# pingcap/tidb

Measured on NVIDIA H100. Metric: hash-join probe rows/sec, higher is better.
Workload: dtype int64

## Files before the change

### tidb_b200/csrc/join.cu

```cuda
#include <memory>
#include <deque>
#include <algorithm>
#include <cmath>
#include <condition_variable>
#include "join_kernels.cuh"
#include "partition_kernels.cuh"
#include "chunk_io.cuh"

namespace tg {

static const int64_t kGeneralBatchRows = 16ll << 20;
static const int64_t kDirectPushRows = 128ll << 10;
static const int64_t kNextWindowRows = 1ll << 20;

struct Side {
  int ncols = 0;
  std::vector<int> types;
  std::vector<uint32_t> flags;
  std::vector<int> elem;
  std::vector<int> kelem;
  bool has_cells = false;
  std::vector<char> needed;
  int key_col = -1;
  std::vector<int> key_cols;
  std::vector<int> key_reject;
  std::vector<int> used;
  DevFilter filter{};
};

struct ColStore {
  std::vector<std::unique_ptr<DevBuf>> data, nulls;
  std::vector<char> has_nulls;
  int64_t rows = 0, cap_rows = 0;
  void init(int ncols) {
    data.clear(); nulls.clear();
    for (int i = 0; i < ncols; i++) { data.emplace_back(new DevBuf()); nulls.emplace_back(new DevBuf()); }
    has_nulls.assign(ncols, 0);
    rows = cap_rows = 0;
  }
  DevCols view(const Side& s) const {
    DevCols v{};
    for (int c = 0; c < s.ncols && c < TG_MAX_COLS; c++) {
      v.data[c] = s.needed[c] ? data[c]->p : nullptr;
      v.nulls[c] = (s.needed[c] && has_nulls[c]) ? nulls[c]->as<uint8_t>() : nullptr;
      v.elem_len[c] = s.elem[c];
    }
    return v;
  }
};

struct ResultBatch {
  std::vector<std::unique_ptr<DevBuf>> cols, bitmaps;
  int64_t rows = 0;
  int64_t consumed = 0;
};

}

using namespace tg;

struct JoinImpl;

struct tg_join {
  std::mutex mu;
  std::mutex res_mu;
  std::condition_variable res_cv;
  std::atomic<bool> closed{false};
  JoinImpl* impl = nullptr;
};

struct JoinImpl : DeviceHandle {
  std::mutex& res_mu;
  std::condition_variable& res_cv;
  explicit JoinImpl(tg_join& shell) : res_mu(shell.res_mu), res_cv(shell.res_cv) {}
  cudaStream_t d2h_stream = nullptr;
  double load_factor = 0.5;
  bool default_load_factor = true;

  int join_type = 0;
  bool build_is_right = true;
  Side build, probe;
  int n_lused = 0, n_rused = 0;
  std::vector<int> lused, rused;
  int probe_kind = PK_INNER;
  bool need_scan = false;
  int scan_mode = 0;
  bool has_flag_col = false;
  int n_out = 0;
  std::vector<int> out_elem;
  std::vector<int> kout_elem;
  KeySpec build_key{}, probe_key{};
  bool multi_key = false;
  DevBuf bkey_syn, bkey_syn_nn, pkey_syn, pkey_syn_nn;
  std::vector<tg_other_item> other;
  std::vector<int> other_build_cols;
  DevOther dev_other{};

  HostStage bstage;
  ColStore bcols;
  bool built = false;
  DevBuf table, rows_store, row_slot, row_rank, slot_used, scalars;
  TableView tv{};
  RowSpec rowspec{};
  std::vector<int> build_word_of_col;
  int u1_payload_col = -1;

  HostStage pstage;
  ColStore pcols_dev;
  DevBuf tmp_cnt, tmp_slot, tmp_off, tmp_sums, out_cursor;
  DevBuf part_scratch;
  DevBuf tile_cnt;
  double seg_match = 1.0;
  int seg_parts = 0;
  int64_t seg_rows = 0, seg_fill_max = 0;
  std::unique_ptr<DevBuf> part_cols[1 + TG_FAST_MAX_PCOLS];
  std::vector<std::unique_ptr<DevBuf>> tmp_valid;
  std::deque<std::unique_ptr<ResultBatch>> results;
  std::vector<std::unique_ptr<ResultBatch>> free_batches;
  std::unique_ptr<ResultBatch> dev_result;
  DevBuf iota;
  int64_t iota_rows = 0;
  std::vector<std::unique_ptr<DevBuf>> out_ids;
  std::atomic<bool> probe_finished{false};
  std::atomic<int64_t> d2h_bytes{0};
  PinBuf win;
  int64_t win_lo = 0, win_hi = 0;
  ResultBatch* win_batch = nullptr;

  tg_join_stats stats{};
};

namespace tg {

static int fill_side(Side& s, int n, const int32_t* types, const uint32_t* flags) {
  if (n <= 0 || n > TG_MAX_COLS) return fail(TG_ERR_UNSUPPORTED, "child schema must have 1..16 columns");
  s.ncols = n;
  s.types.assign(types, types + n);
  s.flags.resize(n);
  for (int i = 0; i < n; i++) s.flags[i] = flags ? flags[i] : 0;
  s.elem.resize(n);
  for (int i = 0; i < n; i++) s.elem[i] = fixed_len(types[i]);
  s.kelem.resize(n);
  for (int i = 0; i < n; i++) s.kelem[i] = s.elem[i] == kCellBytes ? 8 : s.elem[i];
  s.needed.assign(n, 0);
  return TG_OK;
}

static int key_kind_of(int tp) {
  if (is_int_family(tp)) return KEY_I64;
  if (tp == TG_TYPE_DOUBLE) return KEY_F64;
  if (tp == TG_TYPE_FLOAT) return KEY_F32;
  if (tp == TG_TYPE_DATE || tp == TG_TYPE_DATETIME || tp == TG_TYPE_TIMESTAMP) return KEY_TIME;
  return -1;
}
static bool key_unsigned(int tp, uint32_t flag) {
  if (tp == TG_TYPE_YEAR) return true;
  if (tp == TG_TYPE_DURATION) return false;
  return (flag & TG_FLAG_UNSIGNED) != 0;
}

static int check_filter(const Side& s, const tg_filter_item* items, int n, DevFilter& out) {
  if (n < 0 || n > TG_MAX_FILTER) return fail(TG_ERR_UNSUPPORTED, "at most 8 CNF filter items are offloaded");
  out.n = n;
  if (n > 0 && !items) return fail(TG_ERR_INVALID, "filter items are NULL");
  for (int i = 0; i < n; i++) {
    const tg_filter_item& it = items[i];
    if (it.lhs_col < 0 || it.lhs_col >= s.ncols || it.rhs_col >= s.ncols) return fail(TG_ERR_INVALID, "filter column out of range");
    const bool lreal = s.types[it.lhs_col] == TG_TYPE_DOUBLE;
    if ((it.is_real != 0) != lreal || (it.rhs_col >= 0 && (s.types[it.rhs_col] == TG_TYPE_DOUBLE) != lreal))
      return fail(TG_ERR_UNSUPPORTED, "filter compares columns of different families (the planner casts before the filter)");
    if (s.elem[it.lhs_col] != 8 || (it.rhs_col >= 0 && s.elem[it.rhs_col] != 8))
      return fail(TG_ERR_UNSUPPORTED, "filters are offloaded on 8-byte columns only");
    if (it.op < TG_CMP_LT || it.op > TG_CMP_NE) return fail(TG_ERR_INVALID, "bad filter op");
    out.items[i] = it;
  }
  return TG_OK;
}

static int setup(JoinImpl* j, const tg_join_desc* d) {
  if (!d) return fail(TG_ERR_INVALID, "desc is NULL");
  j->join_type = d->join_type;
  j->build_is_right = d->build_is_right != 0;
  Side left, right;
  TG_TRY(fill_side(left, d->n_left_cols, d->left_types, d->left_flags));
  TG_TRY(fill_side(right, d->n_right_cols, d->right_types, d->right_flags));
// ... 152 lines not shown
      TG_TRY(cs.nulls[c]->ensure_preserve(j->device, need, cs.has_nulls[c] ? had : 0, j->stream));
      if (!cs.has_nulls[c]) { TG_CUDA(cudaMemsetAsync(cs.nulls[c]->p, 0xff, had, j->stream)); cs.has_nulls[c] = 1; }
      if (chk->cols[c].null_bitmap) TG_CUDA(cudaMemcpyAsync(cs.nulls[c]->as<uint8_t>() + had, chk->cols[c].null_bitmap, (size_t)((n + 7) / 8), cudaMemcpyDeviceToDevice, j->stream));
      else TG_CUDA(cudaMemsetAsync(cs.nulls[c]->as<uint8_t>() + had, 0xff, (size_t)((n + 7) / 8), j->stream));
    }
  }
  cs.rows += n;
  return TG_OK;
}

static int probe_view(JoinImpl* j, const tg_chunk* chk, DevCols& v) {
  const Side& s = j->probe;
  TG_TRY(device_view(chk, s.ncols, s.needed, s.elem, v));
  for (int c = 0; c < s.ncols; c++)
    if (s.needed[c] && s.elem[c] == kCellBytes && (reinterpret_cast<uintptr_t>(v.data[c]) & 7)) return fail(TG_ERR_INVALID, "DECIMAL device columns must be 8-byte aligned");
  return TG_OK;
}

static int composite_key(JoinImpl* j, const Side& s, const DevCols& v, int64_t n, DevBuf& key, DevBuf& not_null) {
  TG_TRY(key.ensure(j->device, (size_t)(n + 1) * 8 + 16));
  TG_TRY(not_null.ensure(j->device, (size_t)((n + 31) / 32) * 4 + 16));
  if (n <= 0) return TG_OK;
  MultiKeySrc src{};
  src.nk = (int)s.key_cols.size();
  for (int q = 0; q < src.nk; q++) {
    const int c = s.key_cols[q];
    src.data[q] = reinterpret_cast<const int64_t*>(v.data[c]);
    src.nulls[q] = v.nulls[c];
    src.reject[q] = s.key_reject[q];
    if (!src.data[q]) return fail(TG_ERR_INVALID, "key column data is NULL");
  }
  k_composite_key<<<grid_size(j->nsm, n, 256, 8), 256, 0, j->stream>>>(src, n, key.as<int64_t>(), not_null.as<uint32_t>());
  j->stats.kernel_launches++;
  return TG_OK;
}

static int ensure_iota(JoinImpl* j, int64_t rows) {
  if (rows <= j->iota_rows) return TG_OK;
  rows = std::max(rows, 2 * j->iota_rows);
  TG_TRY(j->iota.ensure(j->device, (size_t)rows * 8 + 16));
  k_iota<<<grid_size(j->nsm, rows, 256, 8), 256, 0, j->stream>>>(j->iota.as<int64_t>(), rows);
  j->stats.kernel_launches++;
  j->iota_rows = rows;
  return TG_OK;
}

static int kernel_view(JoinImpl* j, const Side& s, DevCols& v, int64_t rows) {
  if (!s.has_cells) return TG_OK;
  TG_TRY(ensure_iota(j, rows));
  for (int c = 0; c < s.ncols; c++)
    if (s.needed[c] && s.elem[c] == kCellBytes) { v.data[c] = j->iota.p; v.elem_len[c] = 8; }
  return TG_OK;
}

struct ProbeTuning { int ctas_per_sm; bool partition; int parts; int part_min_mb; int part_min_rows; int inplace; };
static ProbeTuning probe_tuning() {
  ProbeTuning t;
  t.ctas_per_sm = env_int("TG_PROBE_CTAS_PER_SM", 0);
  t.partition = env_int("TG_PROBE_PARTITION", 1) != 0;
  t.parts = env_int("TG_PROBE_PARTS", 0);
  t.part_min_mb = env_int("TG_PROBE_PART_MIN_MB", 64);
  t.part_min_rows = env_int("TG_PROBE_PART_MIN_ROWS", 1 << 22);
  t.inplace = env_int("TG_PROBE_INPLACE", -1);
  return t;
}

static size_t l2_slice_target(int device) {
  static size_t cache[64];
  if (device >= 0 && device < 64 && cache[device]) return cache[device];
  int l2 = 0;
  if (cudaDeviceGetAttribute(&l2, cudaDevAttrL2CacheSize, device) != cudaSuccess || l2 <= 0) { cudaGetLastError(); l2 = 50 << 20; }
  const size_t t = (size_t)l2 / 4;
  if (device >= 0 && device < 64) cache[device] = t;
  return t;
}
static int probe_slices(size_t table_bytes, int device, int parts_override) {
  if (parts_override > 0) return std::min(parts_override, TG_MAX_PARTS);
  const size_t target = l2_slice_target(device);
  return (int)std::min<size_t>((table_bytes + target - 1) / target, TG_MAX_PARTS);
}
static const double kMaxDenseLoad = 0.5;
static const double kInplaceMinMatch = 0.995;

static int64_t inplace_seg_cap(const JoinImpl* j, int P, int64_t n_main, int64_t C0) {
  if (j->seg_parts != P || j->seg_rows <= 0) return C0;
  const double f = (double)j->seg_fill_max * (double)n_main / (double)j->seg_rows;
  const int64_t C = ((int64_t)(f + 8.0 * std::sqrt(f)) + 4096 + 127) / 128 * 128;
  return std::min(C, C0);
}

static int build_table(JoinImpl* j) {
  const Side& b = j->build;
  int64_t n = j->bcols.rows;
  j->stats.build_rows = n;
  DevCols bview = j->bcols.view(b);
  TG_TRY(kernel_view(j, b, bview, n));
  KeySpec ks = j->build_key;
  if (j->multi_key) {
    TG_TRY(composite_key(j, b, bview, n, j->bkey_syn, j->bkey_syn_nn));
    ks.data = j->bkey_syn.p; ks.nulls = j->bkey_syn_nn.as<uint8_t>();
  } else { ks.data = bview.data[b.key_col]; ks.nulls = bview.nulls[b.key_col]; }
  unsigned long long nslots = (unsigned long long)((double)(n > 0 ? n : 1) / j->load_factor) + 32;
  if (j->default_load_factor) {
    const unsigned long long fit = ((unsigned long long)TG_MAX_PARTS * (33ull << 20)) / sizeof(Slot);
    const unsigned long long dense = (unsigned long long)((double)(n > 0 ? n : 1) / 0.5) + 32;
    if (nslots > fit) nslots = std::max(fit, dense);
  }
  const unsigned long long align = kHomeWidth;
  nslots &= ~(align - 1);
  if (nslots + 1 >= 0xFFFFFFFFull) return fail(TG_ERR_UNSUPPORTED, "build side too large for 32-bit slot ids");
  TG_TRY(j->table.ensure(j->device, (size_t)(nslots + 2) * sizeof(Slot)));
  TG_TRY(j->row_slot.ensure(j->device, (size_t)(n + 1) * 4));
  TG_TRY(j->row_rank.ensure(j->device, (size_t)(n + 1) * 4));
  TG_TRY(j->scalars.ensure(j->device, 64));
  Slot* slots = j->table.as<Slot>();
  unsigned long long* sc = j->scalars.as<unsigned long long>();
  TG_CUDA(cudaEventRecord(j->ev0, j->stream));
  TG_CUDA(cudaMemsetAsync(sc, 0, 64, j->stream));
  k_table_init<<<grid_size(j->nsm, (int64_t)nslots + 1, 256, 8), 256, 0, j->stream>>>(slots, nslots + 1, nslots);
  j->stats.kernel_launches++;
  if (n > 0) {
    k_build_insert<<<grid_size(j->nsm, n, 256, 8), 256, 0, j->stream>>>(ks, bview, b.filter, n, slots, nslots,
                                                                  j->row_slot.as<uint32_t>(), j->row_rank.as<uint32_t>());
    j->stats.kernel_launches++;
  }
  k_table_stats<<<grid_size(j->nsm, (int64_t)nslots + 1, 256, 8), 256, 0, j->stream>>>(slots, nslots + 1, sc, sc + 1);
  j->stats.kernel_launches++;
  unsigned long long host_sc[3] = {0, 0, 0};
  TG_CUDA(cudaMemcpyAsync(host_sc, sc, 16, cudaMemcpyDeviceToHost, j->stream));
  TG_CUDA(cudaStreamSynchronize(j->stream));
  j->stats.distinct_keys = (int64_t)host_sc[0];
  j->stats.max_dup = (int64_t)host_sc[1];
  j->stats.table_slots = (int64_t)nslots;
  if (host_sc[1] > kCntMask) return fail(TG_ERR_UNSUPPORTED, "a single join key repeats more than 2^28 times on the build side");

  std::vector<int> payload;
  bool key_out = false;
  for (int c : b.used) { if (c == b.key_col) key_out = true; else if (std::find(payload.begin(), payload.end(), c) == payload.end()) payload.push_back(c); }
  bool u1 = host_sc[1] <= 1 && !j->need_scan && payload.size() <= 1 && (!key_out || j->build_key.kind == KEY_I64) && j->other.empty();
  if (u1 && payload.size() == 1) {
    int pc = payload[0];
    if (b.kelem[pc] != 8 || j->bcols.has_nulls[pc]) u1 = false;
  }
  if (u1 && j->default_load_factor && n > 0) {
    const ProbeTuning& tune = probe_tuning();
    const size_t part_min = (size_t)tune.part_min_mb << 20;
    const unsigned long long dense = std::max<unsigned long long>((unsigned long long)TG_MAX_PARTS * l2_slice_target(j->device) / sizeof(Slot),
                                                                  (unsigned long long)((double)n / kMaxDenseLoad) + 32) & ~(align - 1);
    if (tune.partition && nslots * sizeof(Slot) > part_min && dense < nslots && dense * sizeof(Slot) > part_min) {
      nslots = dense;
      j->table.release();
      TG_TRY(j->table.ensure(j->device, (size_t)(nslots + 2) * sizeof(Slot)));
      slots = j->table.as<Slot>();
      k_table_init<<<grid_size(j->nsm, (int64_t)nslots + 1, 256, 8), 256, 0, j->stream>>>(slots, nslots + 1, nslots);
      k_build_insert<<<grid_size(j->nsm, n, 256, 8), 256, 0, j->stream>>>(ks, bview, b.filter, n, slots, nslots,
                                                                    j->row_slot.as<uint32_t>(), j->row_rank.as<uint32_t>());
      j->stats.kernel_launches += 2;
      j->stats.table_slots = (int64_t)nslots;
    }
  }
  j->tv = TableView{slots, nslots, nullptr, 0, -1, TABLE_NONE};
  j->build_word_of_col.assign(b.ncols, -1);
  if (u1) {
    j->u1_payload_col = payload.empty() ? -1 : payload[0];
    if (n > 0) {
      const unsigned long long* pl = j->u1_payload_col >= 0 ? reinterpret_cast<const unsigned long long*>(bview.data[j->u1_payload_col]) : nullptr;
      k_build_scatter_u1<<<grid_size(j->nsm, n, 256, 8), 256, 0, j->stream>>>(j->row_slot.as<uint32_t>(), pl, n, slots);
      j->stats.kernel_launches++;
    }
    j->tv.mode = TABLE_U1;
  } else {
    RowSpec rs{};
    int w = 0;
    bool any_nullable = false;
    std::vector<int> cols;
    for (int c : b.used) if (std::find(cols.begin(), cols.end(), c) == cols.end()) cols.push_back(c);
    for (int c : j->other_build_cols) if (std::find(cols.begin(), cols.end(), c) == cols.end()) cols.push_back(c);
    if ((int)cols.size() + 1 > TG_MAX_COLS) return fail(TG_ERR_UNSUPPORTED, "too many build columns");
    for (int c : cols) {
      rs.col[w] = c; rs.elem_len[w] = b.kelem[c];
      rs.null_bit[w] = j->bcols.has_nulls[c] ? w : -1;
      any_nullable |= j->bcols.has_nulls[c] != 0;
      j->build_word_of_col[c] = w;
      w++;
    }
    rs.null_word = any_nullable ? w : -1;
    rs.nwords = w + (any_nullable ? 1 : 0);
    if (rs.nwords == 0) rs.nwords = 1;
    j->rowspec = rs;
    k_table_assign<<<grid_size(j->nsm, (int64_t)nslots + 1, 256, 8), 256, 0, j->stream>>>(slots, nslots + 1, sc + 2);
    j->stats.kernel_launches++;
    TG_TRY(j->rows_store.ensure(j->device, (size_t)(n + 1) * rs.nwords * 8));
    if (n > 0 && w > 0) {
      k_build_scatter_rows<<<grid_size(j->nsm, n, 256, 8), 256, 0, j->stream>>>(j->row_slot.as<uint32_t>(), j->row_rank.as<uint32_t>(), n, slots,
                                                                          bview, rs, j->rows_store.as<unsigned long long>());
      j->stats.kernel_launches++;
    }
    j->tv.mode = TABLE_G;
    j->tv.rows = j->rows_store.as<unsigned long long>();
    j->tv.row_words = rs.nwords;
    j->tv.null_word = rs.null_word;
    j->dev_other = DevOther{};
    j->dev_other.n = (int)j->other.size();
    for (size_t q = 0; q < j->other.size(); q++) {
      const tg_other_item& it = j->other[q];
      OtherItemDev& o = j->dev_other.it[q];
      o.op = it.op; o.is_real = it.is_real; o.l_unsigned = it.lhs_unsigned; o.r_unsigned = it.rhs_unsigned;
      o.const_i64 = it.const_i64; o.const_f64 = it.const_f64;
      auto operand = [&](int side, int col, int32_t& src, int32_t& idx, int32_t& nbit) {
        nbit = -1;
        if (side < 0) { src = OSRC_CONST; idx = 0; }
        else if (side == 0) { src = OSRC_PROBE; idx = col; }
        else { src = OSRC_BUILD; idx = j->build_word_of_col[col]; nbit = rs.null_bit[idx]; }
      };
      operand(it.lhs_side, it.lhs_col, o.l_src, o.l_idx, o.l_null_bit);
      operand(it.rhs_side, it.rhs_col, o.r_src, o.r_idx, o.r_null_bit);
    }
  }
  if (j->need_scan) {
    TG_TRY(j->slot_used.ensure(j->device, (size_t)nslots + 1));
    TG_CUDA(cudaMemsetAsync(j->slot_used.p, 0, (size_t)nslots + 1, j->stream));
  }
  TG_CUDA(cudaEventRecord(j->ev1, j->stream));
  TG_CUDA(cudaStreamSynchronize(j->stream));
  TG_CUDA(cudaGetLastError());
  j->stats.build_ms = j->elapsed_ms();
  j->stats.table_mode = j->tv.mode;
  j->stats.build_valid_keys = -1;
  j->built = true;
  return TG_OK;
}

static int ensure_result(JoinImpl* j, ResultBatch& rb, int64_t cap_rows, bool preserve, int64_t used_rows) {
  if ((int)rb.cols.size() != j->n_out) {
    rb.cols.clear(); rb.bitmaps.clear();
    for (int i = 0; i < j->n_out; i++) { rb.cols.emplace_back(new DevBuf()); rb.bitmaps.emplace_back(new DevBuf()); }
  }
  if ((int)j->out_ids.size() != j->n_out) {
    j->out_ids.clear();
    for (int i = 0; i < j->n_out; i++) j->out_ids.emplace_back(new DevBuf());
  }
  for (int c = 0; c < j->n_out; c++) {
    size_t bytes = (size_t)(cap_rows + 8) * j->out_elem[c];
    if (preserve) TG_TRY(rb.cols[c]->ensure_preserve(j->device, bytes, (size_t)used_rows * j->out_elem[c], j->stream));
    else TG_TRY(rb.cols[c]->ensure(j->device, bytes));
    if (j->out_elem[c] != kCellBytes) continue;
    if (preserve) TG_TRY(j->out_ids[c]->ensure_preserve(j->device, (size_t)(cap_rows + 8) * 8, (size_t)used_rows * 8, j->stream));
    else TG_TRY(j->out_ids[c]->ensure(j->device, (size_t)(cap_rows + 8) * 8));
  }
  return TG_OK;
}
// ... 104 lines not shown
  std::memset(&fo, 0, sizeof(fo));
  int pcol_of[TG_FAST_MAX_PCOLS];
  for (int c = 0; c < oc.n; c++) {
    const OutSpec& sp = oc.spec[c];
    unsigned long long* dst = reinterpret_cast<unsigned long long*>(oc.data[c]);
    if (sp.src == SRC_BUILD_KEY || (sp.src == SRC_PROBE_COL && sp.idx == j->probe.key_col)) {
      if (fo.n_key_dst >= TG_FAST_MAX_KEYDST) return false;
      fo.key_dst[fo.n_key_dst++] = dst;
    } else if (sp.src == SRC_BUILD_META) {
      if (fo.n_meta_dst >= TG_FAST_MAX_METADST) return false;
      fo.meta_dst[fo.n_meta_dst++] = dst;
    } else if (sp.src == SRC_PROBE_COL) {
      for (int q = 0; q < fo.n_pcols; q++) if (pcol_of[q] == sp.idx) return false;
      if (fo.n_pcols >= TG_FAST_MAX_PCOLS) return false;
      int k = fo.n_pcols++;
      pcol_of[k] = sp.idx;
      fo.psrc[k] = reinterpret_cast<const unsigned long long*>(pview.data[sp.idx]);
      fo.pdst[k] = dst;
    } else return false;
  }
  return true;
}

template <template <int, int, int> class F, typename... A>
static int dispatch_shape(const FastOut& fo, A&&... a) {
#define TG_SHAPE(P, K, M) if (fo.n_pcols == P && fo.n_key_dst == K && fo.n_meta_dst == M) return F<P, K, M>::run(a...);
#define TG_SHAPE_KM(P) TG_SHAPE(P, 0, 0) TG_SHAPE(P, 0, 1) TG_SHAPE(P, 1, 0) TG_SHAPE(P, 1, 1) TG_SHAPE(P, 2, 0) TG_SHAPE(P, 2, 1)
  TG_SHAPE_KM(0) TG_SHAPE_KM(1) TG_SHAPE_KM(2) TG_SHAPE_KM(3)
#undef TG_SHAPE_KM
#undef TG_SHAPE
  return fail(TG_ERR_CUDA, "internal: fused probe shape not instantiated");
}

template <int NPC, int NKD, int NMD>
struct LaunchWarp {
  static int run(JoinImpl* j, const int64_t* pkey, int64_t n, const FastOut& fo, unsigned long long* cur, const ProbeTuning& t, const SegSpec& seg) {
    constexpr int R = 4;
    static int resident = 0;
    if (!resident) {
      int nb = 0;
      if (cudaOccupancyMaxActiveBlocksPerMultiprocessor(&nb, k_probe_inner_u1_w<R, NPC, NKD, NMD>, 256, 0) != cudaSuccess || nb < 1) { cudaGetLastError(); nb = 3; }
      resident = nb;
      if (getenv("TG_DEBUG")) fprintf(stderr, "[tidbgpu] k_probe_inner_u1_w<%d,%d,%d>: %d resident CTAs per SM\n", NPC, NKD, NMD, nb);
    }
    int64_t tiles = (n + 32 * R - 1) / (32 * R);
    int64_t ctas = (tiles + 7) / 8;
    int per_sm = t.ctas_per_sm > 0 ? t.ctas_per_sm : resident;
    int grid = (int)std::min<int64_t>(ctas, (int64_t)j->nsm * per_sm);
    k_probe_inner_u1_w<R, NPC, NKD, NMD><<<grid, 256, 0, j->stream>>>(pkey, n, j->tv, fo, cur, seg);
    return TG_OK;
  }
};
template <int NPC, int NKD, int NMD>
struct LaunchSeg {
  static int run(JoinImpl* j, const int64_t* pkey, int64_t n, const FastOut& fo, unsigned long long* cur, const ProbeTuning& t, const SegSpec& seg) {
    static int resident = 0;
    if (!resident) {
      int nb = 0;
      if (cudaOccupancyMaxActiveBlocksPerMultiprocessor(&nb, k_probe_inner_u1_seg_lean<NPC, NKD, NMD>, 256, 0) != cudaSuccess || nb < 1) { cudaGetLastError(); nb = 3; }
      resident = nb;
    }
    int64_t ctas = (n / 128 + 7) / 8;
    int per_sm = t.ctas_per_sm > 0 ? t.ctas_per_sm : resident;
    int grid = (int)std::min<int64_t>(ctas, (int64_t)j->nsm * per_sm);
    k_probe_inner_u1_seg_lean<NPC, NKD, NMD><<<grid, 256, 0, j->stream>>>(pkey, n, j->tv, fo, cur, seg);
    return TG_OK;
  }
};
template <int NPC, int NKD, int NMD>
struct LaunchInplace {
  static int run(JoinImpl* j, int64_t n, const FastOut& fo, unsigned long long* cur, const ProbeTuning& t, const SegSpec& seg, uint32_t* tile_cnt) {
    if constexpr (NKD == 0) {
      return fail(TG_ERR_CUDA, "internal: the in-place segment probe needs an output fed by the join key");
    } else {
      static int resident = 0;
      if (!resident) {
        int nb = 0;
        if (cudaOccupancyMaxActiveBlocksPerMultiprocessor(&nb, k_probe_inner_u1_seg_inplace<NPC, NKD, NMD>, 256, 0) != cudaSuccess || nb < 1) { cudaGetLastError(); nb = 3; }
        resident = nb;
      }
      int64_t ctas = (n / 128 + 7) / 8;
      int per_sm = t.ctas_per_sm > 0 ? t.ctas_per_sm : resident;
      int grid = (int)std::min<int64_t>(ctas, (int64_t)j->nsm * per_sm);
      k_probe_inner_u1_seg_inplace<NPC, NKD, NMD><<<grid, 256, 0, j->stream>>>(n, j->tv, fo, cur, seg, tile_cnt);
      return TG_OK;
    }
  }
};
static int launch_probe_warp(JoinImpl* j, const int64_t* pkey, int64_t n, const FastOut& fo, unsigned long long* cur, const ProbeTuning& t,
                             const SegSpec& seg = SegSpec{nullptr, 0, 0, 0, nullptr}) {
  j->stats.paths |= TG_JOIN_PATH_PROBE_DIRECT;
  return dispatch_shape<LaunchWarp>(fo, j, pkey, n, fo, cur, t, seg);
}
static int launch_probe_seg(JoinImpl* j, const int64_t* pkey, int64_t n, const FastOut& fo, unsigned long long* cur, const ProbeTuning& t, const SegSpec& seg) {
  j->stats.paths |= TG_JOIN_PATH_PROBE_SEG;
  return dispatch_shape<LaunchSeg>(fo, j, pkey, n, fo, cur, t, seg);
}
static bool aligned16(const void* p) { return (reinterpret_cast<uintptr_t>(p) & 15) == 0; }

static int probe_device(JoinImpl* j, const DevCols& pcells, int64_t n, ResultBatch& rb, bool sync_count, const SegSpec* in_seg = nullptr) {
  const Side& p = j->probe;
  DevCols pview = pcells;
  TG_TRY(kernel_view(j, p, pview, n));
  j->stats.probe_rows += n;
  KeySpec ks = j->probe_key;
  if (j->multi_key) {
    if (in_seg) return fail(TG_ERR_UNSUPPORTED, "segmented device chunks: joins on several key columns take the general path");
    TG_TRY(composite_key(j, p, pview, n, j->pkey_syn, j->pkey_syn_nn));
    ks.data = j->pkey_syn.p; ks.nulls = j->pkey_syn_nn.as<uint8_t>();
  } else { ks.data = pview.data[p.key_col]; ks.nulls = pview.nulls[p.key_col]; }
  TG_TRY(j->out_cursor.ensure(j->device, 64));
  OutCols oc{};
  fill_outspec_probe(j, oc);
  FastOut fo{};
  const bool fast = fast_path_ok(j, pview) && build_fast_out(j, oc, pview, fo);
  if (in_seg && !fast) return fail(TG_ERR_UNSUPPORTED, "segmented device chunks are only accepted by the fused fast path (unique build keys, <= 1 payload, no filters, an output shape the warp kernels cover)");
  if (fast) {
    const ProbeTuning& tune = probe_tuning();
    const int64_t* pkey = reinterpret_cast<const int64_t*>(ks.data);
    const size_t table_bytes = (size_t)j->tv.nslots * sizeof(Slot);
    bool src16 = aligned16(pkey);
    for (int c = 0; c < fo.n_pcols; c++) src16 = src16 && aligned16(fo.psrc[c]);
    const int64_t PTILE = 1024;
    const int64_t n_main = n / PTILE * PTILE;
    int P = 0;
    int64_t C = 0;
    if (n > 0 && tune.partition && src16 && n >= (int64_t)tune.part_min_rows && table_bytes > ((size_t)tune.part_min_mb << 20)) {
      P = probe_slices(table_bytes, j->device, tune.parts);
      C = ((int64_t)((double)n_main / P * 1.05) + 16384 + 127) / 128 * 128;
      if (!(P >= 2 && (int64_t)P * C / 128 < (1ll << 31))) P = 0;
    }
    const bool inplace = P && !in_seg && rb.rows == 0 && fo.n_key_dst >= 1 &&
                         (tune.inplace >= 0 ? tune.inplace != 0 : j->seg_match >= kInplaceMinMatch);
    if (inplace) C = inplace_seg_cap(j, P, n_main, C);
    TG_TRY(ensure_result(j, rb, inplace ? std::max<int64_t>(n, (int64_t)P * C) : rb.rows + n, rb.rows > 0, rb.rows));
    for (int c = 0; c < j->n_out; c++) { oc.data[c] = kernel_out(j, rb, c) + (size_t)rb.rows * 8; oc.valid[c] = nullptr; if (rb.bitmaps[c]->p) rb.bitmaps[c]->release(); }
    build_fast_out(j, oc, pview, fo);
    unsigned long long* cur = j->out_cursor.as<unsigned long long>();
    TG_CUDA(cudaMemsetAsync(cur, 0, 8, j->stream));
    if (n > 0) {
      if (P) {
        const int nc = 1 + fo.n_pcols;
        if (!inplace) {
          for (int c = 0; c < nc; c++) {
            if (!j->part_cols[c]) j->part_cols[c].reset(new DevBuf());
            TG_TRY(j->part_cols[c]->ensure(j->device, (size_t)P * C * 8 + 64));
          }
        }
        TG_TRY(j->part_scratch.ensure(j->device, (size_t)3 * TG_MAX_PARTS * 8 + 64));
        unsigned long long* cursors = j->part_scratch.as<unsigned long long>();
        long long* bases = reinterpret_cast<long long*>(cursors + TG_MAX_PARTS);
        unsigned long long* flag = cursors + 2 * TG_MAX_PARTS;
        PartDst d{};
        d.nparts = P; d.ncols = nc;
        d.src[0] = pkey;
        for (int c = 0; c < fo.n_pcols; c++) d.src[1 + c] = fo.psrc[c];
        for (int c = 0; c < nc; c++)
          for (int q = 0; q < P; q++) d.dst[q][c] = inplace ? (c == 0 ? (void*)fo.key_dst[0] : (void*)fo.pdst[c - 1]) : j->part_cols[c]->p;
        k_segment_bases<<<1, 32, 0, j->stream>>>(cursors, bases, flag, P, C);
        d.dst_base = bases; d.capacity = C; d.overflow = flag;
        if (in_seg) { d.in_cnt = in_seg->cnt; d.in_cap = in_seg->cap; d.in_tiles_per_seg = (uint32_t)(in_seg->cap / PTILE); }
        TG_TRY(launch_partition_scatter<true>(j->device, j->stream, reinterpret_cast<const long long*>(pkey), nullptr, n_main, d, cursors,
                                              &j->stats.kernel_launches, 0, &j->stats.paths));
        const SegSpec seg{cursors, (uint32_t)(C / 128), 0, C, flag};
        if (inplace) {
          const int64_t ntiles = (int64_t)P * C / 128;
// ... 444 lines not shown
```

### tidb_b200/csrc/join_kernels.cuh

```cuda
#pragma once
#include "common.cuh"
#include "tma.cuh"

namespace tg {

struct __align__(16) Slot { int64_t key; unsigned long long meta; };

static const uint32_t kInvalidSlot = 0xFFFFFFFFu;
static const unsigned long long kCntMask = (1ull << 28) - 1;

enum { TABLE_NONE = 0, TABLE_U1 = 1, TABLE_G = 2 };
enum { KEY_I64 = 0, KEY_F64 = 1, KEY_F32 = 2, KEY_TIME = 3 };
enum { SRC_PROBE_COL = 0, SRC_BUILD_KEY = 1, SRC_BUILD_META = 2, SRC_BUILD_WORD = 3, SRC_FLAG = 4 };

struct KeySpec {
  const void* data;
  const uint8_t* nulls;
  int32_t kind;
  int32_t reject_negative;
};

struct TableView {
  Slot* slots;
  unsigned long long nslots;
// ... 614 lines not shown
  const int64_t warps_total = (int64_t)gridDim.x * (blockDim.x >> 5);
  const int64_t warp_id = (int64_t)blockIdx.x * (blockDim.x >> 5) + (threadIdx.x >> 5);
  const int64_t ntiles = n / 128;
  const int64_t* __restrict__ pkey = reinterpret_cast<const int64_t*>(out.key_dst[0]);
  unsigned long long kept = 0;
  for (int64_t tile = warp_id; tile < ntiles; tile += warps_total) {
    const int64_t base = tile * 128;
    const uint32_t p = (uint32_t)tile / seg.tiles_per_seg;
    const unsigned long long c = seg.cnt[p];
    const int64_t limit = (int64_t)p * seg.cap + (int64_t)(c < (unsigned long long)seg.cap ? c : (unsigned long long)seg.cap);
    uint32_t m = 0;
    if (limit - base >= 128) {
      int64_t k[R];
#pragma unroll
      for (int g = 0; g < G; g++) {
        const ulonglong2 kk = __ldcs(reinterpret_cast<const ulonglong2*>(pkey + base + g * 64 + 2 * lane));
        k[2 * g] = (int64_t)kk.x; k[2 * g + 1] = (int64_t)kk.y;
      }
      const bool sentinel = (k[0] == kEmptyKey) | (k[1] == kEmptyKey) | (k[2] == kEmptyKey) | (k[3] == kEmptyKey);
      if (__any_sync(0xffffffffu, sentinel)) {
        m = inplace_tile_generic<NPC, NKD, NMD>(base, limit, t, out, lane);
      } else {
        Slot v[R], w[R];
#pragma unroll
        for (int j = 0; j < R; j++) load_pair(t.slots + home_slot(hash64((uint64_t)k[j]), t.nslots), v[j], w[j]);
        unsigned long long meta[R];
        unsigned hit = 0, run = 0;
#pragma unroll
        for (int j = 0; j < R; j++) {
          meta[j] = 0;
          if (v[j].key == k[j]) { hit |= 1u << j; meta[j] = v[j].meta; }
          else if (w[j].key == k[j]) { hit |= 1u << j; meta[j] = w[j].meta; }
          else if (v[j].key != kEmptyKey && w[j].key != kEmptyKey) run |= 1u << j;
        }
        if (run) {
          uint32_t sl[R];
#pragma unroll
          for (int j = 0; j < R; j++) {
            const unsigned long long s = home_slot(hash64((uint64_t)k[j]), t.nslots) + 2;
            sl[j] = s == t.nslots ? 0u : (uint32_t)s;
          }
          do {
#pragma unroll
            for (int j = 0; j < R; j++) if ((run >> j) & 1u) load_pair(t.slots + sl[j], v[j], w[j]);
#pragma unroll
            for (int j = 0; j < R; j++) {
              if (!((run >> j) & 1u)) continue;
              if (v[j].key == k[j]) { hit |= 1u << j; meta[j] = v[j].meta; run &= ~(1u << j); }
              else if (v[j].key == kEmptyKey) run &= ~(1u << j);
              else if (w[j].key == k[j]) { hit |= 1u << j; meta[j] = w[j].meta; run &= ~(1u << j); }
              else if (w[j].key == kEmptyKey) run &= ~(1u << j);
              else { sl[j] += 2; if (sl[j] == t.nslots) sl[j] = 0; }
            }
          } while (run);
        }
        if (__all_sync(0xffffffffu, hit == 0xFu)) {
          m = 128;
#pragma unroll
          for (int g = 0; g < G; g++) {
            const int64_t o = base + g * 64 + 2 * lane;
            const ulonglong2 kk = make_ulonglong2((unsigned long long)k[2 * g], (unsigned long long)k[2 * g + 1]);
#pragma unroll
            for (int d = 1; d < NKD; d++) __stcs(reinterpret_cast<ulonglong2*>(out.key_dst[d] + o), kk);
#pragma unroll
            for (int d = 0; d < NMD; d++) __stcs(reinterpret_cast<ulonglong2*>(out.meta_dst[d] + o), make_ulonglong2(meta[2 * g], meta[2 * g + 1]));
          }
        } else {
          unsigned long long pv[R][NP];
          inplace_load_pv<NPC>(base, out, pv, lane);
          unsigned bal[R];
#pragma unroll
          for (int j = 0; j < R; j++) {
            bal[j] = __ballot_sync(0xffffffffu, (hit >> j) & 1u);
            m += __popc(bal[j]);
          }
          inplace_store<NPC, NKD, NMD>(base, k, meta, pv, bal, out, lane);
        }
      }
    } else if (limit > base) {
      m = inplace_tile_generic<NPC, NKD, NMD>(base, limit, t, out, lane);
    }
    if (lane == 0) tile_cnt[tile] = m;
    kept += m;
  }
  if (lane == 0 && kept) atomicAdd(out_cursor, kept);
}

__global__ void __launch_bounds__(256)
k_inplace_holes(const uint32_t* __restrict__ tile_cnt, int64_t ntiles, const unsigned long long* out_cursor,
                const unsigned long long* gate, uint32_t* __restrict__ cnt) {
  if (*gate) return;
  const int64_t R = (int64_t)*out_cursor;
  for (int64_t t = blockIdx.x * (int64_t)blockDim.x + threadIdx.x; t < ntiles; t += (int64_t)gridDim.x * blockDim.x) {
    const int64_t s = t * 128, e = s + tile_cnt[t];
    cnt[t] = e < R ? (uint32_t)((s + 128 < R ? s + 128 : R) - e) : 0u;
    cnt[ntiles + t] = e > R ? (uint32_t)(e - (s > R ? s : R)) : 0u;
  }
}

__device__ __forceinline__ int64_t last_le(const unsigned long long* __restrict__ off, int64_t lo, int64_t hi, unsigned long long k) {
  while (lo < hi) {
    const int64_t mid = (lo + hi + 1) >> 1;
    if (off[mid] <= k) lo = mid; else hi = mid - 1;
  }
  return lo;
}

__global__ void __launch_bounds__(256)
k_inplace_fill(const uint32_t* __restrict__ tile_cnt, int64_t ntiles, const unsigned long long* __restrict__ off,
               const unsigned long long* out_cursor, const unsigned long long* gate, FastOut out) {
  if (*gate) return;
  const int lane = threadIdx.x & 31;
  const int64_t warps_total = (int64_t)gridDim.x * (blockDim.x >> 5);
  const int64_t warp_id = (int64_t)blockIdx.x * (blockDim.x >> 5) + (threadIdx.x >> 5);
  const int64_t R = (int64_t)*out_cursor;
  const unsigned long long holes = off[ntiles];
  if (!holes) return;
  for (int64_t t = R / 128 + warp_id; t < ntiles; t += warps_total) {
    const uint32_t c = (uint32_t)(off[ntiles + t + 1] - off[ntiles + t]);
    if (!c) continue;
    const unsigned long long k0 = off[ntiles + t] - holes;
    const int64_t first = t * 128 > R ? t * 128 : R;
    const int64_t lo = last_le(off, 0, ntiles - 1, k0), hi = last_le(off, lo, ntiles - 1, k0 + c - 1);
    for (uint32_t r = lane; r < c; r += 32) {
      const unsigned long long k = k0 + r;
      const int64_t u = last_le(off, lo, hi, k);
      const int64_t dst = u * 128 + tile_cnt[u] + (int64_t)(k - off[u]), src = first + r;
      for (int d = 0; d < out.n_key_dst; d++) out.key_dst[d][dst] = out.key_dst[d][src];
      for (int d = 0; d < out.n_meta_dst; d++) out.meta_dst[d][dst] = out.meta_dst[d][src];
      for (int c2 = 0; c2 < out.n_pcols; c2++) out.pdst[c2][dst] = out.pdst[c2][src];
    }
  }
}

__device__ __forceinline__ bool other_operand(const OtherItemDev& it, bool lhs, const DevCols& pcols, int64_t i, const unsigned long long* brow,
                                              int null_word, unsigned long long& raw) {
  const int src = lhs ? it.l_src : it.r_src, idx = lhs ? it.l_idx : it.r_idx, nbit = lhs ? it.l_null_bit : it.r_null_bit;
  if (src == OSRC_PROBE) {
    const uint8_t* nb = pcols.nulls[idx];
    if (nb && !bit_not_null(nb, i)) return false;
    raw = reinterpret_cast<const unsigned long long*>(pcols.data[idx])[i];
    return true;
  }
  if (src == OSRC_BUILD) {
    if (nbit >= 0 && ((brow[null_word] >> nbit) & 1ull)) return false;
    raw = brow[idx];
    return true;
  }
  raw = it.is_real ? (unsigned long long)__double_as_longlong(it.const_f64) : (unsigned long long)it.const_i64;
  return true;
}
__device__ __forceinline__ bool eval_other(const DevOther& o, const DevCols& pcols, int64_t i, const unsigned long long* brow, int null_word) {
  for (int q = 0; q < o.n; q++) {
    const OtherItemDev& it = o.it[q];
    unsigned long long a, b;
    if (!other_operand(it, true, pcols, i, brow, null_word, a) || !other_operand(it, false, pcols, i, brow, null_word, b)) return false;
    int r = it.is_real ? cmp_real(__longlong_as_double((long long)a), __longlong_as_double((long long)b))
                       : cmp_int((int64_t)a, it.l_unsigned != 0, (int64_t)b, it.r_unsigned != 0);
    if (!apply_cmp(it.op, r)) return false;
  }
  return true;
}

__global__ void __launch_bounds__(256)
k_probe_count(KeySpec key, DevCols pcols, DevFilter filt, DevOther oth, int64_t n, TableView t, int kind,
              uint32_t* __restrict__ row_cnt, uint32_t* __restrict__ row_slot, uint8_t* slot_used) {
// ... 280 lines not shown
```

Before: 28.77 billion.

## Add per-slice perfect-hash index with shared-memory pilots for in-place segment probe

Builds a per-slice perfect-hash index (PTHash-style pilots per bucket) over the dense U1 table. The probe kernel stages each slice's pilot array in shared memory and resolves every key with exactly one slot load. This is meant to replace linear-probing chains and their extra L2 or DRAM traffic. In exchange, build time gets longer because of the many placement kernels, and the probe now runs one persistent 1024-thread block per SM, walking slices sequentially with block-wide syncs. It falls back to the generic path when a key's bucket has no pilot.

New measurement: 31.56 billion (median of 6 runs). 1.1x the previous value.

```diff
diff --git a/tidb_b200/csrc/join.cu b/tidb_b200/csrc/join.cu
--- a/tidb_b200/csrc/join.cu
+++ b/tidb_b200/csrc/join.cu
@@ -101,6 +101,8 @@
   bool built = false;
   DevBuf table, rows_store, row_slot, row_rank, slot_used, scalars;
   TableView tv{};
+  DevBuf pidx_slots, pidx_pilot;
+  SliceIndex pidx{};
   RowSpec rowspec{};
   std::vector<int> build_word_of_col;
   int u1_payload_col = -1;
@@ -419,6 +421,67 @@
 static const double kMaxDenseLoad = 0.5;
 static const double kInplaceMinMatch = 0.995;
 
+static const double kPidxLoad = 0.7;
+static const double kPidxKeysPerBucket = 4.0;
+static const size_t kPidxMaxPilotBytes = 160 << 10;
+static int enqueue_scan(JoinImpl* j, int64_t n, int64_t* nblocks_out);
+static int build_slice_index(JoinImpl* j, const Slot* slots, unsigned long long nslots) {
+  const ProbeTuning& tune = probe_tuning();
+  const uint32_t P = (uint32_t)probe_slices((size_t)nslots * sizeof(Slot), j->device, tune.parts);
+  if (P < 2) return TG_OK;
+  DevBuf cnt;
+  TG_TRY(cnt.ensure(j->device, (size_t)(TG_MAX_PARTS + 1) * 8));
+  unsigned long long* pcnt = cnt.as<unsigned long long>();
+  TG_CUDA(cudaMemsetAsync(pcnt, 0, (size_t)(TG_MAX_PARTS + 1) * 8, j->stream));
+  k_pidx_part_count<<<grid_size(j->nsm, (int64_t)nslots, 256, 8), 256, 0, j->stream>>>(slots, nslots, P, pcnt);
+  unsigned long long hc[TG_MAX_PARTS];
+  TG_CUDA(cudaMemcpyAsync(hc, pcnt, P * 8, cudaMemcpyDeviceToHost, j->stream));
+  TG_CUDA(cudaStreamSynchronize(j->stream));
+  unsigned long long mx = 0;
+  for (uint32_t p = 0; p < P; p++) mx = std::max(mx, hc[p]);
+  SliceIndex ix{};
+  ix.P = P;
+  ix.S = (uint32_t)std::ceil((double)mx / kPidxLoad) + 1;
+  ix.B = ((uint32_t)std::ceil((double)mx / kPidxKeysPerBucket) + 16) & ~15u;
+  int optin = 0;
+  cudaDeviceGetAttribute(&optin, cudaDevAttrMaxSharedMemoryPerBlockOptin, j->device);
+  if (ix.B > kPidxMaxPilotBytes || ix.B > (uint32_t)optin) return TG_OK;
+  const size_t nb = (size_t)P * ix.B, ns = (size_t)P * ix.S;
+  TG_TRY(j->pidx_slots.ensure(j->device, ns * sizeof(Slot)));
+  TG_TRY(j->pidx_pilot.ensure(j->device, nb));
+  DevBuf owner, list;
+  TG_TRY(owner.ensure(j->device, ns * 4));
+  TG_TRY(list.ensure(j->device, (size_t)(mx * P + 1) * 4));
+  TG_TRY(j->tmp_cnt.ensure(j->device, (nb + 1) * 4));
+  Slot* islots = j->pidx_slots.as<Slot>();
+  ix.slots = islots;
+  ix.pilot = j->pidx_pilot.as<uint8_t>();
+  TG_CUDA(cudaMemsetAsync(j->pidx_pilot.p, (int)kPilotNone, nb, j->stream));
+  TG_CUDA(cudaMemsetAsync(owner.p, 0xFF, ns * 4, j->stream));
+  TG_CUDA(cudaMemsetAsync(j->tmp_cnt.p, 0, (nb + 1) * 4, j->stream));
+  k_table_init<<<grid_size(j->nsm, (int64_t)ns, 256, 8), 256, 0, j->stream>>>(islots, ns, ns);
+  const unsigned g = (unsigned)grid_size(j->nsm, (int64_t)nslots, 256, 8);
+  k_pidx_bucket_count<<<g, 256, 0, j->stream>>>(slots, nslots, ix, j->tmp_cnt.as<uint32_t>());
+  int64_t nblocks = 0;
+  TG_TRY(enqueue_scan(j, (int64_t)nb, &nblocks));
+  const unsigned long long* off = j->tmp_off.as<unsigned long long>();
+  k_pidx_lists<<<g, 256, 0, j->stream>>>(slots, nslots, ix, off, j->tmp_cnt.as<uint32_t>(), list.as<uint32_t>());
+  const unsigned gb = (unsigned)grid_size(j->nsm, (int64_t)nb, 256, 8);
+  for (uint32_t size = kPidxMaxBucket; size >= 1; size--)
+    k_pidx_place<<<gb, 256, 0, j->stream>>>(slots, ix, off, list.as<uint32_t>(), size, owner.as<uint32_t>(), j->pidx_pilot.as<uint8_t>());
+  unsigned long long* bad = pcnt + TG_MAX_PARTS;
+  k_pidx_write<<<g, 256, 0, j->stream>>>(slots, nslots, ix, islots, 0, bad);
+  k_pidx_write<<<g, 256, 0, j->stream>>>(slots, nslots, ix, islots, 1, bad);
+  j->stats.kernel_launches += 8 + kPidxMaxBucket;
+  unsigned long long hbad = 0;
+  TG_CUDA(cudaMemcpyAsync(&hbad, bad, 8, cudaMemcpyDeviceToHost, j->stream));
+  TG_CUDA(cudaStreamSynchronize(j->stream));
+  if (hbad) { j->pidx_slots.release(); j->pidx_pilot.release(); return TG_OK; }
+  j->pidx = ix;
+  return TG_OK;
+}
+
+
 static int64_t inplace_seg_cap(const JoinImpl* j, int P, int64_t n_main, int64_t C0) {
   if (j->seg_parts != P || j->seg_rows <= 0) return C0;
   const double f = (double)j->seg_fill_max * (double)n_main / (double)j->seg_rows;
@@ -479,6 +542,9 @@
     int pc = payload[0];
     if (b.kelem[pc] != 8 || j->bcols.has_nulls[pc]) u1 = false;
   }
+  bool sliced = false;
+  j->pidx = SliceIndex{};
+  j->pidx_slots.release(); j->pidx_pilot.release();
   if (u1 && j->default_load_factor && n > 0) {
     const ProbeTuning& tune = probe_tuning();
     const size_t part_min = (size_t)tune.part_min_mb << 20;
@@ -494,6 +560,7 @@
                                                                     j->row_slot.as<uint32_t>(), j->row_rank.as<uint32_t>());
       j->stats.kernel_launches += 2;
       j->stats.table_slots = (int64_t)nslots;
+      sliced = true;
     }
   }
   j->tv = TableView{slots, nslots, nullptr, 0, -1, TABLE_NONE};
@@ -504,6 +571,7 @@
       const unsigned long long* pl = j->u1_payload_col >= 0 ? reinterpret_cast<const unsigned long long*>(bview.data[j->u1_payload_col]) : nullptr;
       k_build_scatter_u1<<<grid_size(j->nsm, n, 256, 8), 256, 0, j->stream>>>(j->row_slot.as<uint32_t>(), pl, n, slots);
       j->stats.kernel_launches++;
+      if (sliced) TG_TRY(build_slice_index(j, slots, nslots));
     }
     j->tv.mode = TABLE_U1;
   } else {
@@ -774,6 +842,16 @@
       int64_t ctas = (n / 128 + 7) / 8;
       int per_sm = t.ctas_per_sm > 0 ? t.ctas_per_sm : resident;
       int grid = (int)std::min<int64_t>(ctas, (int64_t)j->nsm * per_sm);
+      if (j->pidx.P == (uint32_t)(n / seg.cap)) {
+        static bool attr = false;
+        if (!attr) {
+          TG_CUDA(cudaFuncSetAttribute(k_probe_inner_u1_seg_inplace_pidx<NPC, NKD, NMD>, cudaFuncAttributeMaxDynamicSharedMemorySize,
+                                       (int)kPidxMaxPilotBytes));
+          attr = true;
+        }
+        k_probe_inner_u1_seg_inplace_pidx<NPC, NKD, NMD><<<j->nsm, kPidxThreads, j->pidx.B, j->stream>>>(n, j->tv, j->pidx, fo, cur, seg, tile_cnt);
+        return TG_OK;
+      }
       k_probe_inner_u1_seg_inplace<NPC, NKD, NMD><<<grid, 256, 0, j->stream>>>(n, j->tv, fo, cur, seg, tile_cnt);
       return TG_OK;
     }
diff --git a/tidb_b200/csrc/join_kernels.cuh b/tidb_b200/csrc/join_kernels.cuh
--- a/tidb_b200/csrc/join_kernels.cuh
+++ b/tidb_b200/csrc/join_kernels.cuh
@@ -720,6 +720,175 @@
     }
     if (lane == 0) tile_cnt[tile] = m;
     kept += m;
+  }
+  if (lane == 0 && kept) atomicAdd(out_cursor, kept);
+}
+
+static constexpr uint32_t kPilotNone = 255;
+static constexpr int kPidxMaxBucket = 32;
+static constexpr int kPidxThreads = 1024;
+
+struct SliceIndex {
+  const Slot* slots;
+  const uint8_t* pilot;
+  uint32_t P, S, B, pad;
+};
+
+__host__ __device__ __forceinline__ uint32_t pidx_slot(uint64_t h, uint32_t q, uint32_t S) {
+  return slot32(hash64(h ^ ((uint64_t)(q + 1) * 0xC2B2AE3D27D4EB4Full)), S);
+}
+__host__ __device__ __forceinline__ uint32_t pidx_bucket(uint64_t h, uint32_t B) { return mulhi32((uint32_t)h, B); }
+
+__global__ void __launch_bounds__(256) k_pidx_part_count(const Slot* __restrict__ slots, unsigned long long nslots, uint32_t P,
+                                                         unsigned long long* __restrict__ pcnt) {
+  __shared__ unsigned int c[64];
+  for (int i = threadIdx.x; i < 64; i += blockDim.x) c[i] = 0;
+  __syncthreads();
+  for (unsigned long long i = blockIdx.x * (unsigned long long)blockDim.x + threadIdx.x; i < nslots; i += (unsigned long long)gridDim.x * blockDim.x) {
+    const int64_t k = slots[i].key;
+    if (k != kEmptyKey) atomicAdd(&c[slot32(hash64((uint64_t)k), P)], 1u);
+  }
+  __syncthreads();
+  for (int i = threadIdx.x; i < (int)P; i += blockDim.x) if (c[i]) atomicAdd(&pcnt[i], (unsigned long long)c[i]);
+}
+
+__global__ void __launch_bounds__(256) k_pidx_bucket_count(const Slot* __restrict__ slots, unsigned long long nslots, SliceIndex ix,
+                                                           uint32_t* __restrict__ bcnt) {
+  for (unsigned long long i = blockIdx.x * (unsigned long long)blockDim.x + threadIdx.x; i < nslots; i += (unsigned long long)gridDim.x * blockDim.x) {
+    const int64_t k = slots[i].key;
+    if (k == kEmptyKey) continue;
+    const uint64_t h = hash64((uint64_t)k);
+    atomicAdd(&bcnt[(size_t)slot32(h, ix.P) * ix.B + pidx_bucket(h, ix.B)], 1u);
+  }
+}
+
+__global__ void __launch_bounds__(256) k_pidx_lists(const Slot* __restrict__ slots, unsigned long long nslots, SliceIndex ix,
+                                                    const unsigned long long* __restrict__ off, uint32_t* __restrict__ bcnt,
+                                                    uint32_t* __restrict__ list) {
+  for (unsigned long long i = blockIdx.x * (unsigned long long)blockDim.x + threadIdx.x; i < nslots; i += (unsigned long long)gridDim.x * blockDim.x) {
+    const int64_t k = slots[i].key;
+    if (k == kEmptyKey) continue;
+    const uint64_t h = hash64((uint64_t)k);
+    const size_t b = (size_t)slot32(h, ix.P) * ix.B + pidx_bucket(h, ix.B);
+    list[off[b] + atomicSub(&bcnt[b], 1u) - 1] = (uint32_t)i;
+  }
+}
+
+__global__ void __launch_bounds__(256) k_pidx_place(const Slot* __restrict__ slots, SliceIndex ix, const unsigned long long* __restrict__ off,
+                                                    const uint32_t* __restrict__ list, uint32_t size, uint32_t* __restrict__ owner,
+                                                    uint8_t* __restrict__ pilot) {
+  const size_t nb = (size_t)ix.P * ix.B;
+  for (size_t b = blockIdx.x * (size_t)blockDim.x + threadIdx.x; b < nb; b += (size_t)gridDim.x * blockDim.x) {
+    const unsigned long long o = off[b];
+    if (off[b + 1] - o != size) continue;
+    uint64_t h[kPidxMaxBucket];
+    for (uint32_t j = 0; j < size; j++) h[j] = hash64((uint64_t)slots[list[o + j]].key);
+    uint32_t* const base = owner + (b / ix.B) * ix.S;
+    for (uint32_t q = 0; q < kPilotNone; q++) {
+      uint32_t won = 0;
+      for (; won < size; won++)
+        if (atomicCAS(base + pidx_slot(h[won], q, ix.S), 0xFFFFFFFFu, (uint32_t)b) != 0xFFFFFFFFu) break;
+      if (won == size) { pilot[b] = (uint8_t)q; break; }
+      for (uint32_t j = 0; j < won; j++) atomicExch(base + pidx_slot(h[j], q, ix.S), 0xFFFFFFFFu);
+    }
+  }
+}
+
+__global__ void __launch_bounds__(256) k_pidx_write(const Slot* __restrict__ slots, unsigned long long nslots, SliceIndex ix,
+                                                    Slot* __restrict__ islots, int check, unsigned long long* __restrict__ bad) {
+  for (unsigned long long i = blockIdx.x * (unsigned long long)blockDim.x + threadIdx.x; i < nslots; i += (unsigned long long)gridDim.x * blockDim.x) {
+    const Slot s = slots[i];
+    if (s.key == kEmptyKey) continue;
+    const uint64_t h = hash64((uint64_t)s.key);
+    const uint32_t p = slot32(h, ix.P);
+    const uint32_t q = ix.pilot[(size_t)p * ix.B + pidx_bucket(h, ix.B)];
+    if (q == kPilotNone) continue;
+    Slot* d = islots + (size_t)p * ix.S + pidx_slot(h, q, ix.S);
+    if (!check) *d = s;
+    else if (d->key != s.key || d->meta != s.meta) atomicAdd(bad, 1ull);
+  }
+}
+
+template <int NPC, int NKD, int NMD>
+__global__ void __launch_bounds__(kPidxThreads, 1)
+k_probe_inner_u1_seg_inplace_pidx(int64_t n, TableView t, SliceIndex ix, FastOut out, unsigned long long* __restrict__ out_cursor,
+                                  SegSpec seg, uint32_t* __restrict__ tile_cnt) {
+  static_assert(NKD >= 1, "the probe key is read from the first key destination");
+  constexpr int R = 4, G = 2, NP = NPC > 0 ? NPC : 1;
+  extern __shared__ __align__(16) uint8_t spil[];
+  if (seg.gate && ((*seg.gate != 0ull) != (seg.gate_want != 0))) return;
+  const int lane = threadIdx.x & 31;
+  const int64_t warps_total = (int64_t)gridDim.x * (kPidxThreads / 32);
+  const int64_t warp_id = (int64_t)blockIdx.x * (kPidxThreads / 32) + (threadIdx.x >> 5);
+  const int64_t* __restrict__ pkey = reinterpret_cast<const int64_t*>(out.key_dst[0]);
+  const int nseg = (int)(n / 128 / seg.tiles_per_seg);
+  unsigned long long kept = 0;
+  for (int p = 0; p < nseg; p++) {
+    __syncthreads();
+    const uint4* src = reinterpret_cast<const uint4*>(ix.pilot + (size_t)p * ix.B);
+    for (uint32_t i = threadIdx.x; i < ix.B / 16; i += kPidxThreads) reinterpret_cast<uint4*>(spil)[i] = __ldcs(src + i);
+    __syncthreads();
+    const unsigned long long c = seg.cnt[p];
+    const int64_t limit = (int64_t)p * seg.cap + (int64_t)(c < (unsigned long long)seg.cap ? c : (unsigned long long)seg.cap);
+    const int64_t t0 = (int64_t)p * seg.tiles_per_seg, t1 = t0 + seg.tiles_per_seg;
+    const Slot* __restrict__ islots = ix.slots + (size_t)p * ix.S;
+    for (int64_t tile = t0 + warp_id; tile < t1; tile += warps_total) {
+      const int64_t base = tile * 128;
+      uint32_t m = 0;
+      if (limit - base >= 128) {
+        int64_t k[R];
+#pragma unroll
+        for (int g = 0; g < G; g++) {
+          const ulonglong2 kk = __ldcs(reinterpret_cast<const ulonglong2*>(pkey + base + g * 64 + 2 * lane));
+          k[2 * g] = (int64_t)kk.x; k[2 * g + 1] = (int64_t)kk.y;
+        }
+        uint32_t q[R];
+        bool generic = false;
+#pragma unroll
+        for (int j = 0; j < R; j++) {
+          q[j] = spil[pidx_bucket(hash64((uint64_t)k[j]), ix.B)];
+          generic |= (k[j] == kEmptyKey) | (q[j] == kPilotNone);
+        }
+        if (__any_sync(0xffffffffu, generic)) {
+          m = inplace_tile_generic<NPC, NKD, NMD>(base, limit, t, out, lane);
+        } else {
+          unsigned long long meta[R];
+          unsigned hit = 0;
+#pragma unroll
+          for (int j = 0; j < R; j++) {
+            const Slot v = load_slot(islots + pidx_slot(hash64((uint64_t)k[j]), q[j], ix.S));
+            meta[j] = v.meta;
+            if (v.key == k[j]) hit |= 1u << j;
+          }
+          if (__all_sync(0xffffffffu, hit == 0xFu)) {
+            m = 128;
+#pragma unroll
+            for (int g = 0; g < G; g++) {
+              const int64_t o = base + g * 64 + 2 * lane;
+              const ulonglong2 kk = make_ulonglong2((unsigned long long)k[2 * g], (unsigned long long)k[2 * g + 1]);
+#pragma unroll
+              for (int d = 1; d < NKD; d++) __stcs(reinterpret_cast<ulonglong2*>(out.key_dst[d] + o), kk);
+#pragma unroll
+              for (int d = 0; d < NMD; d++) __stcs(reinterpret_cast<ulonglong2*>(out.meta_dst[d] + o), make_ulonglong2(meta[2 * g], meta[2 * g + 1]));
+            }
+          } else {
+            unsigned long long pv[R][NP];
+            inplace_load_pv<NPC>(base, out, pv, lane);
+            unsigned bal[R];
+#pragma unroll
+            for (int j = 0; j < R; j++) {
+              bal[j] = __ballot_sync(0xffffffffu, (hit >> j) & 1u);
+              m += __popc(bal[j]);
+            }
+            inplace_store<NPC, NKD, NMD>(base, k, meta, pv, bal, out, lane);
+          }
+        }
+      } else if (limit > base) {
+        m = inplace_tile_generic<NPC, NKD, NMD>(base, limit, t, out, lane);
+      }
+      if (lane == 0) tile_cnt[tile] = m;
+      kept += m;
+    }
   }
   if (lane == 0 && kept) atomicAdd(out_cursor, kept);
 }
```
